# hellobertrand/zxc

Measured on NVIDIA H100. Metric: decompress GB/s (uncompressed), higher is better.
Workload: dtype u8

## Files before the change

include/zxc_b200.h:

```cpp
#ifndef ZXC_B200_H
#define ZXC_B200_H

#include <stddef.h>
#include <stdint.h>

#include "zxc_export.h"
#include "zxc_opts.h"

#ifdef __cplusplus
extern "C" {
#endif

typedef struct {
    uint64_t src_off;
    uint64_t dst_off;
    uint32_t src_len;
    uint32_t dst_cap;
} zxc_b200_job_t;

typedef struct {
    uint64_t decoded_size;
    uint32_t block_size;
    uint32_t n_blocks;
    uint32_t dict_id;
// ... 12 lines not shown
ZXC_EXPORT int zxc_b200_decode_blocks(const void* d_src, void* d_dst, const zxc_b200_job_t* d_jobs,
                                      uint32_t n_jobs, int32_t* d_status, const void* d_dict,
                                      uint32_t dict_size, const void* d_dict_huf, void* d_scratch,
                                      size_t scratch_size, uint32_t block_size,
                                      int verify_checksums, void* stream);

ZXC_EXPORT int64_t zxc_b200_reduce_status(const int32_t* d_status, const zxc_b200_job_t* d_jobs,
                                          uint32_t n_jobs, void* stream);

ZXC_EXPORT size_t zxc_b200_encode_scratch_size(uint64_t src_size, const zxc_compress_opts_t* opts);

ZXC_EXPORT int zxc_b200_compress_device(const void* d_src, uint64_t src_size, void* d_dst, uint64_t dst_capacity,
                                        const zxc_compress_opts_t* opts, void* d_scratch, size_t scratch_size,
                                        int64_t* d_result, zxc_b200_job_t* d_jobs, void* stream);

ZXC_EXPORT size_t zxc_b200_decompress_device_scratch_size(uint64_t dst_capacity, uint32_t block_size);

ZXC_EXPORT int zxc_b200_decompress_device(const void* d_src, uint64_t src_size, void* d_dst, uint64_t dst_capacity,
                                          const zxc_decompress_opts_t* opts, void* d_scratch, size_t scratch_size,
                                          int64_t* d_result, void* stream);

ZXC_EXPORT uint64_t zxc_b200_launch_count(void);

ZXC_EXPORT int zxc_b200_train_phase_times(double* ms, int n);

#ifdef __cplusplus
}
#endif
#endif
```

profiles/occupancy_probe.py:

```python
import argparse
import ctypes as C
import os
import re
import shutil
import subprocess
import sys
import tempfile
import time

ROOT = os.path.dirname(os.path.dirname(os.path.abspath(__file__)))
sys.path.insert(0, os.path.join(ROOT, "tests"))
sys.path.insert(0, ROOT)

VARIANTS = [
    ("parent", "parent", "", {}, "baseline: lean at 7 CTAs, 72 registers"),
    ("pad7", "pad7", "-DLEAN_SMEM_PAD=2048u", {}, "7 CTAs, 164 KB carve-out: the L1 shrink alone"),
    ("reg64_7", "reg64_7", "-DLEAN_CTAS_PER_SM=8u -DLEAN_CARVEOUT=57", {},
     "64-register build, 132 KB carve-out hint, so 7 CTAs if the driver follows the hint: the spills alone"),
    ("cta8", "cta8", "-DLEAN_CTAS_PER_SM=8u", {}, "8 CTAs, 64 registers, 164 KB carve-out: both"),
    ("cta8_grid7", "cta8", "-DLEAN_CTAS_PER_SM=8u", {"ZXC_B200_DECODE_CTAS": "7"},
     "the 8-CTA build with a 7-CTA grid: spills and the L1 shrink, without the eighth CTA"),
    ("parent_grid6", "parent", "", {"ZXC_B200_DECODE_CTAS": "6"}, "the lean instance's own 6 -> 7 CTA step"),
    ("ring2k_7", "ring2k_7", "-DRING_BYTES=2048u", {}, "7 CTAs, 2 KiB rings"),
    ("ring2k_8", "ring2k_8", "-DRING_BYTES=2048u -DLEAN_CTAS_PER_SM=8u", {},
     "8 CTAs, 2 KiB rings: more warps at a 100 KB carve-out"),
]
LEAN = "_Z17zxc_decode_kernelILb0ELb0ELb0ELb1EEv12DecodeParams"


def build(out_dir, nvextra):
    lib = os.path.join(out_dir, "libzxc.so.4")
    if not os.path.exists(lib):
        subprocess.run(["make", "-j", str(os.cpu_count() or 4), f"NVEXTRA={nvextra}", f"OUT={out_dir}"],
                       cwd=os.path.join(ROOT, "zxc_b200", "csrc"), check=True, stdout=subprocess.DEVNULL)
    return lib


def lean_resources(out_dir):
    log = open(os.path.join(out_dir, "obj", "ptxas.log")).read()
    blk = log.split(f"Compiling entry function '{LEAN}'")[1].split("Compiling entry function")[0]
    sp = re.search(r"(\d+) bytes spill stores, (\d+) bytes spill loads", blk)
    return int(re.search(r"Used (\d+) registers", blk).group(1)), int(sp.group(1)), int(sp.group(2))


def card():
    q = "name,power.limit,clocks.max.sm,clocks.sm"
    r = subprocess.run(["nvidia-smi", f"--query-gpu={q}", "--format=csv,noheader"], stdout=subprocess.PIPE, text=True)
    return r.stdout.strip().splitlines()[0] if r.returncode == 0 and r.stdout.strip() else "nvidia-smi unavailable"


class Runner:
    def __init__(self, path, dev, d_src, d_dst, d_jobs, d_status, nb):
        import bench
        import torch

        lib = C.CDLL(path)
        lib.zxc_b200_decode_scratch_size.restype = C.c_size_t
        lib.zxc_b200_decode_scratch_size.argtypes = [C.c_uint32]
        lib.zxc_b200_decode_blocks.restype = C.c_int
        lib.zxc_b200_decode_blocks.argtypes = [C.c_void_p, C.c_void_p, C.c_void_p, C.c_uint32, C.c_void_p,
                                               C.c_void_p, C.c_uint32, C.c_void_p, C.c_void_p, C.c_size_t,
                                               C.c_uint32, C.c_int, C.c_void_p]
        self.lib, self.nb, self.block = lib, nb, bench.BLOCK
        self.bufs = (d_src, d_dst, d_jobs, d_status)
        self.scratch_size = lib.zxc_b200_decode_scratch_size(bench.BLOCK)
        self.d_scratch = torch.empty(self.scratch_size, dtype=torch.uint8, device=dev)
        self.stream = torch.cuda.current_stream(dev)

    def step(self):
        d_src, d_dst, d_jobs, d_status = self.bufs
        rc = self.lib.zxc_b200_decode_blocks(d_src.data_ptr(), d_dst.data_ptr(), d_jobs.data_ptr(), self.nb,
                                             d_status.data_ptr(), None, 0, None, self.d_scratch.data_ptr(),
                                             self.scratch_size, self.block, 0, self.stream.cuda_stream)
        assert rc == 0, rc

    def time(self, steps):
        import torch

        e0, e1 = torch.cuda.Event(enable_timing=True), torch.cuda.Event(enable_timing=True)
        e0.record(self.stream)
        for _ in range(steps):
            self.step()
        e1.record(self.stream)
        e1.synchronize()
        return e0.elapsed_time(e1) / steps


def main():
    ap = argparse.ArgumentParser()
    ap.add_argument("--out", help="build directory (default: a temporary one)")
# ... 34 lines not shown
    prod.zxc_b200_plan_frame.restype = C.c_int64
    prod.zxc_b200_plan_frame.argtypes = [C.c_void_p, C.c_size_t, C.c_void_p, C.c_size_t, C.c_void_p]
    nb = prod.zxc_b200_plan_frame(frame.ctypes.data, frame.size, None, 0, None)
    jobs = np.zeros(nb * C.sizeof(bench.Job), dtype=np.uint8)
    assert prod.zxc_b200_plan_frame(frame.ctypes.data, frame.size, jobs.ctypes.data, nb, None) == nb
    dev = torch.device("cuda", 0)
    d_src = torch.from_numpy(frame).to(dev)
    d_dst = torch.empty(data.size, dtype=torch.uint8, device=dev)
    d_jobs = torch.from_numpy(jobs).to(dev)
    d_status = torch.empty(nb, dtype=torch.int32, device=dev)
    want = torch.from_numpy(data).to(dev)
    runners = {}
    for name, _, _, env, _ in variants:
        r = Runner(libs[name], dev, d_src, d_dst, d_jobs, d_status, nb)
        d_dst.zero_()
        os.environ.update(env)
        for _ in range(3):
            r.step()
        torch.cuda.synchronize(dev)
        for k in env:
            del os.environ[k]
        assert torch.equal(d_dst, want), f"{name}: decoded bytes differ"
        runners[name] = r
    del want
    rates = {v[0]: [] for v in variants}
    for k in range(args.rounds):
        for name in rates:
            runners[name].time(2)
            ms = runners[name].time(args.steps)
            rates[name].append(data.size / ms / 1e6)
        print(f"round {k + 1}: " + ", ".join(f"{n} {rates[n][-1]:.1f}" for n in rates), flush=True)
        time.sleep(0.5)
    print(f"\ncard after the runs: {card()}")
    base = np.median(rates[variants[0][0]])
    print(f"\n| variant | GB/s decoded, per round | median | spread | against {variants[0][0]} |")
    print("|---|---|---|---|---|")
    for name in rates:
        v = rates[name]
        med = float(np.median(v))
        print(f"| {name} | {' / '.join(f'{x:.1f}' for x in v)} | {med:.1f} | {100 * (max(v) - min(v)) / med:.2f} % | "
              f"{100 * (med / base - 1):+.1f} % |")


if __name__ == "__main__":
    main()
```

zxc_b200/csrc/zxc_decode.cuh:

```cuda
#pragma once
#include <cuda_runtime.h>
#include <stdint.h>

#include "zxc_b200.h"
#include "zxc_error.h"

typedef uint8_t u8;
typedef uint32_t u32;
typedef uint64_t u64;
typedef int32_t i32;

#define FULL 0xFFFFFFFFu
#ifndef ZXC_FASTMOD
#define ZXC_FASTMOD 1
#endif
#ifndef ZXC_TAIL_SMEM
#define ZXC_TAIL_SMEM 1
#endif
#ifndef ZXC_ALIGNED_LD
#define ZXC_ALIGNED_LD 1
#endif
#ifndef ZXC_HINTS
#define ZXC_HINTS 0
#endif
#if ZXC_HINTS
#define ZXC_RARE(x) __builtin_expect(!!(x), 0)
#else
#define ZXC_RARE(x) (x)
#endif
#ifndef ZXC_STAT
#define ZXC_STAT(i, v)
#endif
#ifndef WARPS_PER_CTA
#define WARPS_PER_CTA 4
#endif
#define CTA_THREADS (WARPS_PER_CTA * 32)
#ifndef RING_BYTES
#define RING_BYTES 4096u
#endif
#define RING_LIMIT (RING_BYTES - 576u)
#ifndef CTAS_PER_SM
#define CTAS_PER_SM 7u
#endif
#ifndef LEAN_CTAS_PER_SM
#define LEAN_CTAS_PER_SM CTAS_PER_SM
#endif
#ifndef LEAN_SMEM_PAD
#define LEAN_SMEM_PAD 0u
#endif

#define BT_RAW 0
#define BT_GLO 1
#define BT_GHI 2
#define BT_EOF 255

#define FLAG_VERIFY 1u
#define FLAG_UNITS_ON 4u
#define FLAG_UNITS_OFF 8u
#define FLAG_DEFERRED 2u
#define D2_DEFER_STATUS ((i32)0x80000000)

struct DecodeParams {
    const u8* src;
    u8* dst;
    const zxc_b200_job_t* jobs;
    i32* status;
    const u8* dict;
    const u8* dict_huf;
    u8* scratch;
    unsigned long long* counter;
    u32 n_jobs;
    u32 dict_size;
    u32 scratch_stride;
    u32 flags;
    u32 block_cap;
    u32* defer_list;
    u32* defer_count;
    u32 defer_cap;
};

__device__ __forceinline__ u32 ld16(const u8* p) { return (u32)p[0] | ((u32)p[1] << 8); }
__device__ __forceinline__ u32 ld32(const u8* p) {
    return (u32)p[0] | ((u32)p[1] << 8) | ((u32)p[2] << 16) | ((u32)p[3] << 24);
}
__device__ __forceinline__ u64 ld64(const u8* p) { return (u64)ld32(p) | ((u64)ld32(p + 4) << 32); }

__device__ __forceinline__ u32 warp_incl_scan(u32 v, u32 lane) {
#pragma unroll
    for (int d = 1; d < 32; d <<= 1) {
        const u32 t = __shfl_up_sync(FULL, v, d);
        if (lane >= (u32)d) v += t;
    }
    return v;
}

#ifdef __CUDACC__
__device__ __forceinline__ u32 smem_addr(const void* p) {
    u32 a = (u32)__cvta_generic_to_shared(p);
    asm volatile("" : "+r"(a));
    return a;
}
template <int OFF> __device__ __forceinline__ void sts32(u32 a, u32 v) {
    asm volatile("st.shared.u32 [%0+%2], %1;" ::"r"(a), "r"(v), "n"(OFF) : "memory");
}
template <int OFF> __device__ __forceinline__ void sts16(u32 a, u32 v) {
    asm volatile("st.shared.u16 [%0+%2], %1;" ::"r"(a), "h"((unsigned short)v), "n"(OFF) : "memory");
}
template <int OFF> __device__ __forceinline__ void sts8(u32 a, u32 v) {
    asm volatile("st.shared.u8 [%0+%2], %1;" ::"r"(a), "r"(v), "n"(OFF) : "memory");
}
#else
extern u8 smem[];
static inline u32 smem_addr(const void* p) { return (u32)(reinterpret_cast<const u8*>(p) - smem); }
template <int OFF> static inline void sts32(u32 a, u32 v) { memcpy(smem + a + OFF, &v, 4); }
template <int OFF> static inline void sts16(u32 a, u32 v) { const unsigned short h = (unsigned short)v; memcpy(smem + a + OFF, &h, 2); }
template <int OFF> static inline void sts8(u32 a, u32 v) { smem[a + OFF] = (u8)v; }
#endif

#ifdef __CUDACC__
__device__ __forceinline__ void prefetch_l1(const void* p) { asm volatile("prefetch.global.L1 [%0];" ::"l"(p)); }
#else
static inline void prefetch_l1(const void*) {}
#endif

#if ZXC_TRACE
#define TRACE_SLOTS 16
#define TRACE_ROWS 8192
enum {
    TR_UNPACK, TR_SCAN, TR_LIT, TR_MATCH, TR_TAIL, TR_FLUSH, TR_START, TR_END, TR_GIANT, TR_CLAIM,
    TR_BATCHES, TR_BLOCKS, TR_M_RING, TR_M_GLOBAL, TR_M_DICT, TR_M_SEQ
};
__device__ unsigned long long zxc_trace_acc[TRACE_ROWS * TRACE_SLOTS];
__device__ __forceinline__ void trace_add(u32 slot, unsigned long long v, u32 lane) {
    const u32 row = blockIdx.x * WARPS_PER_CTA + (threadIdx.x >> 5);
    if (lane == 0 && row < TRACE_ROWS) atomicAdd(&zxc_trace_acc[row * TRACE_SLOTS + slot], v);
}
// ... 215 lines not shown
                if (lit_comp > avail) return ZXC_ERROR_CORRUPT_DATA;
                const int rc = rle_expand(p_data, lit_comp, scratch, n_lit, lane);
                if (rc != ZXC_OK) return rc;
                __syncwarp();
                S.lit = scratch;
                S.n_lit_avail = n_lit;
            } else {
                S.lit = p_data;
                S.n_lit_avail = 0;
            }
        } else if (enc_lit == 0) {
            S.lit = p_data;
            S.n_lit_avail = lit_comp;
        } else {
            return ZXC_ERROR_CORRUPT_DATA;
        }
        const u64 sz_off = enc_off ? (u64)n_seq : (u64)n_seq * 2;
        const u64 consumed = (u64)lit_comp + tok_comp + sz_off;
        if (consumed > avail) return ZXC_ERROR_CORRUPT_DATA;
        if (avail - lit_comp < 32) return ZXC_ERROR_CORRUPT_DATA;
        if (enc_tok != 0 && enc_tok != 2) return ZXC_ERROR_CORRUPT_DATA;
        S.tok = p_data + lit_comp;
        S.offs = S.tok + tok_comp;
        if (!LEAN && enc_tok == 2) {
            if (n_seq == 0 || n_seq > block_cap / 5u + 16u || tok_comp < 128) return ZXC_ERROR_CORRUPT_DATA;
            const int rc = pivco_decode(S.tok, S.tok + 128, tok_comp - 128, tok_buf, n_seq, hw, cum, cum_words, lane);
            if (rc != ZXC_OK) return rc;
            __syncwarp();
            S.tok = tok_buf;
        }
        S.ext = S.offs + (u32)sz_off;
        S.ext_end = avail - (u32)consumed;
    } else {
        if (enc_lit != 0 || enc_tok != 0) return ZXC_ERROR_CORRUPT_DATA;
        const u32 avail = comp - 12;
        const u64 consumed = (u64)n_lit + (u64)n_seq * 4;
        if (consumed > avail) return ZXC_ERROR_CORRUPT_DATA;
        if (avail - n_lit < 32) return ZXC_ERROR_CORRUPT_DATA;
        S.lit = pay + 12;
        S.n_lit_avail = n_lit;
        S.tok = S.lit + n_lit;
        S.ext = S.tok + (size_t)n_seq * 4;
        S.ext_end = avail - (u32)consumed;
    }
    return ZXC_OK;
}
// ... 209 lines not shown
            const u32 m = (u32)(reinterpret_cast<uintptr_t>(bp)) & 3u;
            const u32* wp = reinterpret_cast<const u32*>(bp - m) + w0;
            const u32 dw = ring_s + (pj & 0xFFFFu) - da + 4u * w0;
            const u32 sh = m * 8u;
            const u32 left = lfe - w0;
            const u32 nsrc = left + (m ? 1u : 0u);
            u32 W[5];
#pragma unroll
            for (int i = 0; i < 5; i++) W[i] = (u32)i < nsrc ? wp[i] : 0u;
            sts32<0>(dw, __funnelshift_r(W[0], W[1], sh));
            if (1 < left) sts32<4>(dw, __funnelshift_r(W[1], W[2], sh));
            if (2 < left) sts32<8>(dw, __funnelshift_r(W[2], W[3], sh));
            if (3 < left) sts32<12>(dw, __funnelshift_r(W[3], W[4], sh));
        }
    }
}

#ifndef ZXC_NW
#define ZXC_NW 8
#endif
#define LIT_SHORT (4u * ZXC_NW - 4u)
#define MATCH_SHORT (4u * ZXC_NW - 4u)

template <bool UNITS, bool GHI, bool HAS_DICT, bool LEAN>
__device__ int decode_lz_block(const u8* pay, u32 comp, u8* out, u32 cap, const u8* dict_in,
                               u32 dict_size_in, const u8* dict_huf, u8* scratch, u32 scratch_cap, u8* ring,
                               u32 lane, u32 P_flags) {
    constexpr bool ghi = GHI;
    const u8* dict = HAS_DICT ? dict_in : (const u8*)0;
    const u32 dict_size = HAS_DICT ? dict_size_in : 0u;
    ZXC_TRACE_DECL;
    ZXC_TRACE_ADD(TR_BLOCKS, 1, lane);
    Sections S;
    const int prc = parse_sections<LEAN>(pay, comp, ghi, cap, dict_huf, scratch, scratch_cap, lane, S);
    if (prc != ZXC_OK) return prc;
    const u8* lit = S.lit;
    const u8* tok = S.tok;
    const u8* offs = S.offs;
    const u8* ext = S.ext;
    const u32 ext_end = S.ext_end, n_lit_avail = S.n_lit_avail, n_seq = S.n_seq, enc_off = S.enc_off;

    (void)P_flags;
    if (UNITS && cap <= 65536u) {
        u8* tok_buf = scratch + scr_lit_cap(scratch_cap);
        u8* hw_area = tok_buf + scr_tok_cap(scratch_cap);
        const bool scratch_busy = (lit == scratch) || (tok == tok_buf);
        u8* tab = scratch_busy ? hw_area : scratch;
        const u32 tab_bytes = scratch_busy ? (u32)HUF_WORK_BYTES + scr_cum_cap(scratch_cap)
                                           : scr_stride(scratch_cap) - 256u;
        const int r = decode_lz_units(lit, n_lit_avail, tok, offs, ext, ext_end, n_seq, enc_off, ghi, out, cap, dict,
                                      dict_size, tab, tab_bytes, lane);
        if (r != UW_NOT_TAKEN) return r;
    }

    const u32 mask = RING_BYTES - 1;
    const u32 esc = ghi ? 255u : 15u;
    const u32 lt_mask = (1u << lane) - 1u;
    const bool al16 = (reinterpret_cast<uintptr_t>(out) & 15u) == 0;
    Window w;
    w.ring = ring;
    w.out = out;
    w.dict = dict;
    w.dict_size = dict_size;
    w.near_lo = 0;
    const u32 ring_s = smem_addr(ring);
    (void)ring_s;
    u32 O = 0, L = 0, F = 0, epos = 0, ring_lo = 0;

    u32* vals = reinterpret_cast<u32*>(scratch + scr_lit_cap(scratch_cap) + scr_tok_cap(scratch_cap) + (u32)HUF_WORK_BYTES);
    if constexpr (LEAN) {
        if (4ull * ext_end > scr_cum_cap(scratch_cap)) return D2_DEFER_STATUS;
    }
    const bool use_vals = LEAN || (ext_end != 0u && 4ull * ext_end <= scr_cum_cap(scratch_cap));
    u32 n_val = 0, ord_base = 0;
    if (use_vals && (!LEAN || ext_end != 0u)) {
        const u32 seg = max(4u, (ext_end + 31u) / 32u);
        const u32 nseg = (ext_end + seg - 1u) / seg;
        const u32 lo = lane * seg, hi = min(ext_end, lo + seg);
        u64 inc = lane < nseg ? z2_seg_map(ext, lo, hi, ext_end) : Z2_MAP_ID;
#pragma unroll
        for (int dd = 1; dd < 32; dd <<= 1) {
            const u64 o = __shfl_up_sync(FULL, inc, dd);
            if (lane >= (u32)dd) inc = z2_map_compose(o, inc);
        }
        u64 excl = __shfl_up_sync(FULL, inc, 1);
        if (lane == 0) excl = Z2_MAP_ID;
        n_val = z2_map_cnt(__shfl_sync(FULL, inc, 31), 0);
        if (lane < nseg) {
            const u32 ent = z2_map_exit(excl, 0);
            if (ent != 3u) z2_seg_values(ext, lo, hi, ext_end, ent, z2_map_cnt(excl, 0), vals);
        }
        __syncwarp();
// ... 45 lines not shown
                    b = enc_off ? (u32)offs[i] : ld16(offs + 2 * (size_t)i);
                } else if (enc_off) {
                    b = lds8(st_o.ring_s + ((ox0 + i) & (ST_RING - 1u)));
                } else {
                    const u32 x = ox0 + 2u * i;
                    b = (ox0 & 1u) ? (lds8(st_o.ring_s + (x & (ST_RING - 1u))) |
                                      (lds8(st_o.ring_s + ((x + 1u) & (ST_RING - 1u))) << 8))
                                   : lds16(st_o.ring_s + (x & (ST_RING - 1u)));
                }
            } else if (t_st) {
                const u32 x = tx0 + 4u * i;
                if (tx0 & 3u) {
                    a = lds8(st_t.ring_s + (x & (ST_RING - 1u))) | (lds8(st_t.ring_s + ((x + 1u) & (ST_RING - 1u))) << 8) |
                        (lds8(st_t.ring_s + ((x + 2u) & (ST_RING - 1u))) << 16) |
                        (lds8(st_t.ring_s + ((x + 3u) & (ST_RING - 1u))) << 24);
                } else {
                    a = lds32(st_t.ring_s + (x & (ST_RING - 1u)));
                }
            } else {
                a = ld32(tok + 4 * (size_t)i);
            }
#else
            if (!ghi) {
                a = tok[i];
#if ZXC_ALIGNED_LD
                if (LEAN) {
                    const u32 oi = n_seq + (enc_off ? i : 2u * i);
                    if (enc_off) b = (u32)tok[oi];
                    else if ((reinterpret_cast<uintptr_t>(tok) + n_seq) & 1u) b = ld16(tok + oi);
                    else b = (u32)*reinterpret_cast<const unsigned short*>(tok + oi);
                } else if (enc_off) b = (u32)offs[i];
                else if (reinterpret_cast<uintptr_t>(offs) & 1u) b = ld16(offs + 2 * (size_t)i);
                else b = (u32)reinterpret_cast<const unsigned short*>(offs)[i];
#else
                b = enc_off ? (u32)offs[i] : ld16(offs + 2 * (size_t)i);
#endif
            } else {
#if ZXC_ALIGNED_LD
                a = (reinterpret_cast<uintptr_t>(tok) & 3u) ? ld32(tok + 4 * (size_t)i) : reinterpret_cast<const u32*>(tok)[i];
#else
                a = ld32(tok + 4 * (size_t)i);
#endif
            }
#endif
            if (!ghi) {
                ll = a >> 4;
                ml = a & 15;
                off = b + 1;
            } else {
                ll = a >> 24;
                ml = (a >> 16) & 0xFF;
                off = (a & 0xFFFF) + 1;
            }
        }
        const bool e_ll = valid && ll == esc, e_ml = valid && ml == esc;
        const u32 m_ll = __ballot_sync(FULL, e_ll), m_ml = __ballot_sync(FULL, e_ml);
        ZXC_TRACE_MARK(TR_UNPACK, lane);
        u32 k_esc = 0, epos_end = epos;
        if ((m_ll | m_ml) && use_vals) {
            u32 k = ord_base + __popc(m_ll & lt_mask) + __popc(m_ml & lt_mask);
            if (e_ll) {
                ll += k < n_val ? vals[k] : 0u;
                k++;
            }
            if (e_ml) ml += k < n_val ? vals[k] : 0u;
        } else if (ZXC_RARE((m_ll | m_ml) != 0)) {
            const u32 ord_ll = __popc(m_ll & lt_mask) + __popc(m_ml & lt_mask);
            k_esc = __popc(m_ll) + __popc(m_ml);
            u32 my_pos = ext_end;
            for (u32 s = 0; s < k_esc; s++) {
                if (s == ord_ll) my_pos = epos_end;
                epos_end = varint_advance(ext, epos_end, ext_end);
            }
            if (e_ll) ll += read_varint(ext, my_pos, ext_end);
            if (e_ml) ml += read_varint(ext, my_pos, ext_end);
        }
        if (valid) ml += 5;
        const u32 tot = ll + ml;
        const u32 s_ll = warp_incl_scan(ll, lane);
        const u32 s_tot = warp_incl_scan(tot, lane);

        const u32 nvalid = min(32u, n_seq - base);
        const u32 m = __popc(__ballot_sync(FULL, valid && s_tot <= RING_LIMIT));
        const u32 lit_start = L + s_ll - ll;
        const u32 out_start = O + s_tot - tot;
        const u32 mdst = out_start + ll;

        if (ZXC_RARE(m == 0)) {
            const u32 g_ll = __shfl_sync(FULL, ll, 0), g_ml = __shfl_sync(FULL, ml, 0),
                      g_off = __shfl_sync(FULL, off, 0);
            ZXC_STAT(9, 1);
            if (L + g_ll > n_lit_avail || (u64)O + g_ll + g_ml > cap) {
                ST_CLOSE();
                return ZXC_ERROR_OVERFLOW;
            }
            if (O + g_ll + dict_size < g_off) {
                ST_CLOSE();
                return ZXC_ERROR_BAD_OFFSET;
            }
            __syncwarp();
            ring_flush(w, F, O, lane, al16);
            __syncwarp();
            flush_wait(lane);
            warp_copy(out + O, lit + L, g_ll, lane);
            __syncwarp();
            warp_match_global(w, O + g_ll, g_off, g_ml, lane);
            __syncwarp();
            O += g_ll + g_ml;
            L += g_ll;
            F = O;
            ring_lo = O >= 64 ? O - 64 : 0;
            for (u32 p = ring_lo + lane; p < O; p += 32) ring[p & mask] = out[p];
            __syncwarp();
            const u32 q = ((m_ll & 1u) ? 1u : 0u) + ((m_ml & 1u) ? 1u : 0u);
            ord_base += q;
            if (!use_vals)
                for (u32 s = 0; s < q; s++) epos = varint_advance(ext, epos, ext_end);
            base += 1;
            ZXC_TRACE_MARK(TR_GIANT, lane);
            continue;
        }

        ZXC_STAT(10, m < nvalid);
        ZXC_STAT(11, m < nvalid && !use_vals);
        const bool act = lane < m;
        const bool ovf = act && (lit_start + ll > n_lit_avail || out_start + tot > cap);
        const bool bad = act && (mdst + dict_size < off);
        const u32 m_err = __ballot_sync(FULL, ovf || bad);
        if (ZXC_RARE(m_err != 0)) {
            ZXC_STAT(19, 1);
            const int code = ovf ? ZXC_ERROR_OVERFLOW : ZXC_ERROR_BAD_OFFSET;
            ST_CLOSE();
            return __shfl_sync(FULL, code, __ffs(m_err) - 1);
        }
        const u32 T = __shfl_sync(FULL, s_tot, m - 1), TL = __shfl_sync(FULL, s_ll, m - 1);
#if ZXC_STAGE && ZXC_STAGE_LIT
        const u32 lx0 = (u32)(reinterpret_cast<uintptr_t>(lit) & 15u);
        const StWindow lw = LitStream::need(stage_s, lit, lx0 + L, lx0 + L + TL, 8u, lane);
#endif
        {
            const i32 a = (i32)(O + T) - (i32)RING_BYTES + 32;
            w.near_lo = a > (i32)ring_lo ? a : (i32)ring_lo;
        }

        flush_wait(lane);
        const i32 src_lo = (i32)mdst - (i32)off;
        const i32 src_end = min((i32)mdst, src_lo + (i32)ml);
        const bool near = src_lo >= w.near_lo;
        const u32 si = (u32)src_lo & mask;
        const bool in_dict = src_lo + (i32)ml + 8 <= 0 && (i32)dict_size + src_lo >= 8;
        const bool m_word_ok = ((mdst & mask) + ml + 4 <= RING_BYTES) &&
                               (near ? (si >= 8 && si + ml + 8 <= RING_BYTES)
                                     : (in_dict || (src_lo >= 8 && src_lo + (i32)ml + 4 <= w.near_lo)));
        const bool m_lane_ok = m_word_ok && ml <= MATCH_SHORT && off >= ml;
        const bool m_grp_ok = m_word_ok && !m_lane_ok && off >= ml;
        const u8* m_sp = near ? ring + si : (src_lo < 0 ? dict + ((i32)dict_size + src_lo) : out + src_lo);
        const bool l_word_ok = (out_start & mask) + ll + 4 <= RING_BYTES;

        const bool m_free = src_end <= (i32)O;
        if (LEAN && !HAS_DICT && act && m_free && !near && src_lo >= 0) {
            const u8* ps = out + src_lo;
            const u8* pe = ps + ml - 1u;
            prefetch_l1(ps);
            if ((reinterpret_cast<uintptr_t>(ps) ^ reinterpret_cast<uintptr_t>(pe)) >> 7) prefetch_l1(pe);
        }
        ZXC_TRACE_ADD(TR_M_RING, __popc(__ballot_sync(FULL, act && near)), lane);
        ZXC_TRACE_ADD(TR_M_GLOBAL, __popc(__ballot_sync(FULL, act && !near && src_lo >= 0)), lane);
        ZXC_TRACE_ADD(TR_M_DICT, __popc(__ballot_sync(FULL, act && !near && src_lo < 0)), lane);
        ZXC_TRACE_ADD(TR_M_SEQ, __popc(__ballot_sync(FULL, act && !m_free)), lane);
        ZXC_TRACE_ADD(TR_BATCHES, 1, lane);
        ZXC_TRACE_MARK(TR_SCAN, lane);
        ZXC_STAT(0, 1);
        ZXC_STAT(1, m);
        bool lit_pass = true;
#pragma unroll 1
        for (;;) {
            bool ready, lok, gok;
            u32 it_d, it_n;
            const u8* it_sp;
            if (lit_pass) {
                ready = act && ll > 0;
                it_d = out_start;
                it_n = ll;
                it_sp = lit + lit_start;
#if ZXC_STAGE && ZXC_STAGE_LIT
                {
                    const u8* sp_s = lit_ptr(lw, lx0 + lit_start, ll);
                    if (sp_s) it_sp = sp_s;
                    ZXC_STAT(13, __popc(__ballot_sync(FULL, ready && sp_s != 0)));
                    ZXC_STAT(14, __popc(__ballot_sync(FULL, ready)));
                }
#endif
                lok = l_word_ok && ll <= LIT_SHORT;
                gok = l_word_ok && ll > LIT_SHORT;
            } else {
                ready = act && m_free;
                it_d = mdst;
                it_n = ml;
                it_sp = m_sp;
                lok = m_lane_ok;
                gok = m_grp_ok;
            }
            lane_copy_words2<ZXC_NW>(ring_s, it_d, it_sp, it_n, ready && lok);
            const u32 m_grp = __ballot_sync(FULL, ready && gok);
            ZXC_STAT(2, 1);
            ZXC_STAT(3, __popc(__ballot_sync(FULL, ready && lok)));
            ZXC_STAT(4, __popc(m_grp));
            ZXC_STAT(5, m_grp != 0);
            ZXC_STAT(6, __popc(__ballot_sync(FULL, ready && !lok && !gok)));
            ZXC_STAT(7, __ballot_sync(FULL, ready && lok) != 0);
            ZXC_STAT(17, __popc(__ballot_sync(FULL, !lit_pass && ready && (lok || gok) && src_lo < 0)));
            ZXC_STAT(18, __popc(__ballot_sync(FULL, !lit_pass && ready && !lok && !gok)));
            ZXC_STAT(20, __popc(__ballot_sync(FULL, !lit_pass && ready && (lok || gok) && near)));
            ZXC_STAT(21, __popc(__ballot_sync(FULL, !lit_pass && ready && (lok || gok) && !near && src_lo >= 0)));
            if (m_grp) balanced_copy_words(ring_s, m_grp, it_d, it_sp, it_n, lane);
            u32 m_slow = __ballot_sync(FULL, ready && !lok && !gok);
            while (ZXC_RARE(m_slow != 0)) {
                const int j = __ffs(m_slow) - 1;
                m_slow &= m_slow - 1;
                const u32 d = __shfl_sync(FULL, it_d, j), n = __shfl_sync(FULL, it_n, j);
                const u32 aux = __shfl_sync(FULL, lit_pass ? lit_start : off, j);
                if (lit_pass) {
                    for (u32 k = lane; k < n; k += 32) ring[(d + k) & mask] = lit[aux + k];
                } else {
                    warp_match_to_ring(w, d, aux, n, lane);
                }
            }
            __syncwarp();
            ZXC_TRACE_MARK(lit_pass ? TR_LIT : TR_MATCH, lane);
            if (!lit_pass) break;
            lit_pass = false;
        }
        {
            u32 rest = __ballot_sync(FULL, act && !m_free);
            const u32 my_pk = ml | ((near && off >= ml) ? 0x80000000u : 0u);
            ZXC_STAT(12, __popc(rest));
            while (rest) {
                const int j = __ffs(rest) - 1;
                rest &= rest - 1;
                const u32 d = __shfl_sync(FULL, mdst, j), pk = __shfl_sync(FULL, my_pk, j);
                const u32 n = pk & 0x7FFFFFFFu;
                if (pk >> 31) {
                    const u32 sl = __shfl_sync(FULL, (u32)src_lo, j);
#if ZXC_TAIL_SMEM
                    for (u32 k = lane; k < n; k += 32) sts8<0>(ring_s + ((d + k) & mask), lds8(ring_s + ((sl + k) & mask)));
#else
                    for (u32 k = lane; k < n; k += 32) ring[(d + k) & mask] = ring[(sl + k) & mask];
#endif
                } else {
                    warp_match_to_ring(w, d, __shfl_sync(FULL, off, j), n, lane);
                }
                __syncwarp();
            }
        }
        ZXC_TRACE_MARK(TR_TAIL, lane);

        O += T;
        L += TL;
        ring_flush(w, F, O & ~511u, lane, al16);
        __syncwarp();
        ZXC_TRACE_MARK(TR_FLUSH, lane);

        if (m < nvalid) {
            const u32 below = (1u << m) - 1u;
            const u32 q = __popc(m_ll & below) + __popc(m_ml & below);
            ord_base += q;
            if (!use_vals)
                for (u32 s = 0; s < q; s++) epos = varint_advance(ext, epos, ext_end);
            base += m;
        } else {
            ord_base += __popc(m_ll) + __popc(m_ml);
            epos = epos_end;
            base += 32;
        }
    }

    ST_LIT_CLOSE();
    const u32 rem = n_lit_avail - L;
    if (rem > cap - O) return ZXC_ERROR_OVERFLOW;
    ring_flush(w, F, O, lane, al16);
    __syncwarp();
    flush_wait(lane);
    warp_copy(out + O, lit + L, rem, lane);
    ZXC_TRACE_MARK(TR_END, lane);
    return (int)(O + rem);
}

template <bool UNITS, bool HAS_DICT, bool LEAN = false>
__device__ int decode_job(const DecodeParams& P, const zxc_b200_job_t& job, u8* scratch, u8* ring, u32 lane) {
    const u8* blk = P.src + job.src_off;
    u8* out = P.dst + job.dst_off;
    if (job.src_len < 8) return LEAN ? D2_DEFER_STATUS : ZXC_ERROR_SRC_TOO_SMALL;
    const u32 type = blk[0];
    const u32 comp = ld32(blk + 3);
    const bool verify = (P.flags & FLAG_VERIFY) != 0;
    if (LEAN) {
        const bool whole = !verify && (u64)job.src_len >= 8ull + comp;
        const bool take = whole && (type == BT_RAW || (type == BT_GLO && comp >= 12u && blk[8 + 9] == 0 && blk[8 + 8] <= 1));
        if (!take) return D2_DEFER_STATUS;
    }
    if ((u64)job.src_len < 8ull + comp + (verify ? 4u : 0u)) return ZXC_ERROR_SRC_TOO_SMALL;
    const u8* data = blk + 8;
    if constexpr (!LEAN) {
        if (verify && ld32(data + comp) != warp_checksum(data, comp, lane)) return ZXC_ERROR_BAD_CHECKSUM;
    }
    switch (type) {
        case BT_GLO:
            return decode_lz_block<UNITS, false, HAS_DICT, LEAN>(data, comp, out, job.dst_cap, P.dict, P.dict_size,
                                                                 P.dict_huf, scratch, P.block_cap, ring, lane, P.flags);
        case BT_GHI:
            if constexpr (LEAN) return D2_DEFER_STATUS;
            else return decode_lz_block<UNITS, true, HAS_DICT, false>(data, comp, out, job.dst_cap, P.dict, P.dict_size,
                                                                      P.dict_huf, scratch, P.block_cap, ring, lane, P.flags);
        case BT_RAW:
            if (comp > job.dst_cap) return ZXC_ERROR_DST_TOO_SMALL;
            warp_copy(out, data, comp, lane);
            return (int)comp;
        case BT_EOF:
            return ZXC_ERROR_CORRUPT_DATA;
        default:
            return ZXC_ERROR_BAD_BLOCK_TYPE;
    }
}

template <bool UNITS, bool DEFERRED, bool HAS_DICT, bool LEAN>
__global__ void __launch_bounds__(CTA_THREADS, LEAN ? LEAN_CTAS_PER_SM : CTAS_PER_SM) zxc_decode_kernel(const DecodeParams P) {
    extern __shared__ __align__(16) u8 smem[];
    const u32 lane = threadIdx.x & 31;
    const u32 wic = threadIdx.x >> 5;
    const u32 gwarp = blockIdx.x * WARPS_PER_CTA + wic;
    u8* scratch = P.scratch + (size_t)gwarp * P.scratch_stride + 256;
    u8* ring = smem + (size_t)wic * WARP_SMEM_BYTES;
#if ZXC_STAGE
    st_init(smem_addr(ring) + RING_BYTES, lane);
#endif
    if (DEFERRED) {
        const u32 n_def = *P.defer_count;
        if (n_def == 0) return;
        if (n_def <= P.defer_cap) {
            for (;;) {
                unsigned long long k = 0;
                if (lane == 0) k = atomicAdd(P.counter, 1ull);
                k = __shfl_sync(FULL, k, 0);
                if (k >= n_def) break;
                const u32 j = P.defer_list[k];
                const zxc_b200_job_t job = P.jobs[j];
                const int r = decode_job<UNITS, HAS_DICT, false>(P, job, scratch, ring, lane);
                flush_wait(lane);
                __syncwarp();
                if (lane == 0) P.status[j] = r;
            }
            return;
        }
        for (;;) {
            unsigned long long b = 0;
            if (lane == 0) b = atomicAdd(P.counter, 32ull);
            b = __shfl_sync(FULL, b, 0);
            if (b >= P.n_jobs) break;
            const unsigned long long jj = b + lane;
            u32 m = __ballot_sync(FULL, jj < P.n_jobs && P.status[jj] == D2_DEFER_STATUS);
            while (m) {
                const unsigned long long j = b + (u32)(__ffs(m) - 1);
                m &= m - 1;
                const zxc_b200_job_t job = P.jobs[j];
                const int r = decode_job<UNITS, HAS_DICT, false>(P, job, scratch, ring, lane);
                flush_wait(lane);
                __syncwarp();
                if (lane == 0) P.status[j] = r;
            }
        }
        return;
    }
    for (;;) {
        ZXC_TRACE_DECL;
        unsigned long long j = 0;
        if (lane == 0) j = atomicAdd(P.counter, 1ull);
        j = __shfl_sync(FULL, j, 0);
        ZXC_TRACE_MARK(TR_CLAIM, lane);
        if (j >= P.n_jobs) break;
        const zxc_b200_job_t job = P.jobs[j];
        const int r = decode_job<UNITS, HAS_DICT, LEAN>(P, job, scratch, ring, lane);
        flush_wait(lane);
        __syncwarp();
        if (lane == 0) {
            P.status[j] = r;
            if (LEAN && r == D2_DEFER_STATUS) {
                const u32 slot = atomicAdd(P.defer_count, 1u);
                if (slot < P.defer_cap) P.defer_list[slot] = (u32)j;
            }
        }
    }
}

__global__ void zxc_reduce_kernel(const i32* status, const zxc_b200_job_t* jobs, u32 n,
                                  unsigned long long* out ) {
    const u32 i = blockIdx.x * blockDim.x + threadIdx.x;
    unsigned long long bad = ~0ull, sum = 0;
    if (i < n) {
        const i32 s = status[i];
        if (s < 0 || (u32)s != jobs[i].dst_cap) bad = i;
        else sum = (u32)s;
    }
    for (int d = 16; d >= 1; d >>= 1) {
        const unsigned long long ob = __shfl_xor_sync(FULL, bad, d);
// ... 9 lines not shown
```

zxc_b200/csrc/zxc_gpu.cu:

```cuda
#include <cuda_runtime.h>
#include <stdint.h>
#include <stdio.h>
#include <stdlib.h>
#include <string.h>
#include <pthread.h>

#include "zxc_error.h"
#include "zxc_gpu.h"

#include "zxc_decode.cuh"
#include "zxc_decode2.cuh"
#include "zxc_encode.cuh"
#include "zxc_assemble.cuh"
#include "zxc_dplan.cuh"
#include "zxc_train.cuh"

static pthread_once_t g_once = PTHREAD_ONCE_INIT;
static int g_init_rc = ZXC_B200_ERROR_NO_DEVICE;
static int g_sm_count = 0;
static unsigned long long g_launches = 0;
static pthread_mutex_t g_pool_mu = PTHREAD_MUTEX_INITIALIZER;

#define PIN_CHUNK ((size_t)32 << 20)

// ... 256 lines not shown
    int dev = 0;
    cudaGetDevice(&dev);
    cudaDeviceProp prop;
    if (cudaGetDeviceProperties(&prop, dev) != cudaSuccess) {
        g_init_rc = ZXC_B200_ERROR_CUDA;
        return;
    }
    g_sm_count = prop.multiProcessorCount;
    g_init_rc = ZXC_OK;
}

extern "C" int zxg_init(void) {
    pthread_once(&g_once, init_once);
    return g_init_rc;
}

extern "C" int zxc_b200_device_count(void) {
    int n = 0;
    if (cudaGetDeviceCount(&n) != cudaSuccess) return 0;
    return n;
}

extern "C" uint64_t zxc_b200_launch_count(void) { return g_launches; }

#if ZXC_TRACE
extern "C" ZXC_EXPORT int zxc_b200_trace_read(unsigned long long* host) {
    const size_t bytes = sizeof(unsigned long long) * TRACE_ROWS * TRACE_SLOTS;
    if (cudaDeviceSynchronize() != cudaSuccess) return -1;
    if (cudaMemcpyFromSymbol(host, zxc_trace_acc, bytes) != cudaSuccess) return -1;
    void* d = 0;
    if (cudaGetSymbolAddress(&d, zxc_trace_acc) != cudaSuccess || cudaMemset(d, 0, bytes) != cudaSuccess) return -1;
    if (cudaDeviceSynchronize() != cudaSuccess) return -1;
    return TRACE_ROWS * TRACE_SLOTS;
}
#endif

extern "C" int zxg_current_device(void) {
    int dev = 0;
    if (cudaGetDevice(&dev) != cudaSuccess) {
        cudaGetLastError();
        return 0;
    }
    return dev;
}
extern "C" int zxg_device_count(void) { return zxc_b200_device_count(); }
extern "C" int zxg_set_device(int dev) {
// ... 279 lines not shown
    P.src = (const u8*)d_src;
    P.dst = (u8*)d_dst;
    P.jobs = d_jobs;
    P.status = d_status;
    P.dict = (const u8*)d_dict;
    P.dict_huf = (const u8*)d_dict_huf;
    P.scratch = (u8*)d_scratch;
    P.counter = d_counter;
    P.n_jobs = n_jobs;
    P.dict_size = d_dict ? dict_size : 0;
    P.scratch_stride = scratch_stride_for(block_size);
    P.flags = verify ? FLAG_VERIFY : 0;
    {
        static int units_mode = -2;
        if (units_mode == -2) {
            const char* e = getenv("ZXC_B200_UNITS");
            units_mode = e ? (e[0] == '1' ? 1 : 0) : -1;
        }
        if (units_mode == 1) P.flags |= FLAG_UNITS_ON;
        if (units_mode == 0) P.flags |= FLAG_UNITS_OFF;
    }
    const bool units = (P.flags & FLAG_UNITS_ON) != 0;
    P.block_cap = block_size;
    const int grid = grid_for(n_jobs);
    const size_t warp_scratch = (size_t)grid * WARPS_PER_CTA * P.scratch_stride;
    if (warp_scratch > scratch_size) return ZXC_ERROR_MEMORY;
    if (!preset && cudaMemsetAsync(d_counter, 0, 3 * sizeof(unsigned long long), st) != cudaSuccess)
        return ZXC_B200_ERROR_CUDA;
    size_t off = (warp_scratch + 255) & ~(size_t)255;
    P.defer_count = (u32*)(d_counter + 2);
    P.defer_cap = off + (size_t)DEFER_CAP * 4 <= scratch_size ? DEFER_CAP : 0u;
    P.defer_list = (u32*)((u8*)d_scratch + off);
    D2Config c;
    if (!verify && d2_config(block_size, &c)) {
        static int attr_done_smem = 0;
        if (attr_done_smem < (int)c.smem) {
            if (cudaFuncSetAttribute(zxc_decode2_kernel, cudaFuncAttributeMaxDynamicSharedMemorySize, 233472 - 1024) !=
                cudaSuccess)
                return ZXC_B200_ERROR_CUDA;
            attr_done_smem = 233472;
        }
        Decode2Params Q;
        Q.src = P.src;
        Q.dst = P.dst;
        Q.jobs = d_jobs;
        Q.status = d_status;
        Q.dict = P.dict;
// ... 55 lines not shown
        }
        P.flags |= FLAG_DEFERRED;
        P.counter = d_counter + 1;
    }
    const bool has_dict = P.dict != NULL && P.dict_size != 0;
    if (!verify && !units && !(P.flags & FLAG_DEFERRED)) {
#ifdef LEAN_CARVEOUT
        static int carveout_done = 0;
        if (!carveout_done) {
            cudaFuncSetAttribute(zxc_decode_kernel<false, false, true, true>,
                                 cudaFuncAttributePreferredSharedMemoryCarveout, LEAN_CARVEOUT);
            cudaFuncSetAttribute(zxc_decode_kernel<false, false, false, true>,
                                 cudaFuncAttributePreferredSharedMemoryCarveout, LEAN_CARVEOUT);
            carveout_done = 1;
        }
#endif
        const u32 lean_smem = DECODE_SMEM_BYTES + LEAN_SMEM_PAD;
        if (has_dict) zxc_decode_kernel<false, false, true, true><<<grid, CTA_THREADS, lean_smem, st>>>(P);
        else zxc_decode_kernel<false, false, false, true><<<grid, CTA_THREADS, lean_smem, st>>>(P);
        __atomic_add_fetch(&g_launches, 1, __ATOMIC_RELAXED);
        if (cudaGetLastError() != cudaSuccess) return ZXC_B200_ERROR_CUDA;
        P.flags |= FLAG_DEFERRED;
        P.counter = d_counter + 1;
    }
    if (P.flags & FLAG_DEFERRED) {
        if (has_dict) zxc_decode_kernel<false, true, true, false><<<grid, CTA_THREADS, DECODE_SMEM_BYTES, st>>>(P);
        else zxc_decode_kernel<false, true, false, false><<<grid, CTA_THREADS, DECODE_SMEM_BYTES, st>>>(P);
    } else if (units) {
        if (has_dict) zxc_decode_kernel<true, false, true, false><<<grid, CTA_THREADS, DECODE_SMEM_BYTES, st>>>(P);
        else zxc_decode_kernel<true, false, false, false><<<grid, CTA_THREADS, DECODE_SMEM_BYTES, st>>>(P);
    } else {
        if (has_dict) zxc_decode_kernel<false, false, true, false><<<grid, CTA_THREADS, DECODE_SMEM_BYTES, st>>>(P);
        else zxc_decode_kernel<false, false, false, false><<<grid, CTA_THREADS, DECODE_SMEM_BYTES, st>>>(P);
    }
    __atomic_add_fetch(&g_launches, 1, __ATOMIC_RELAXED);
    return cudaGetLastError() == cudaSuccess ? ZXC_OK : ZXC_B200_ERROR_CUDA;
}

static int launch_decode(const void* d_src, void* d_dst, const zxc_b200_job_t* d_jobs, u32 n_jobs,
                         i32* d_status, const void* d_dict, u32 dict_size, const void* d_dict_huf,
                         void* d_scratch, size_t scratch_size, u32 block_size, int verify,
                         unsigned long long* d_counter, cudaStream_t st) {
    return launch_decode_ex(d_src, d_dst, d_jobs, n_jobs, d_status, d_dict, dict_size, d_dict_huf, d_scratch,
                            scratch_size, block_size, verify, d_counter, st, 0);
}

// ... 1046 lines not shown
```

Baseline: 395.0.

## Run lean decode kernel at 8 CTAs per SM by trimming live registers

Raises the lean decode kernel's launch bound from 7 to 8 CTAs per SM. To fit the tighter register budget without spills, it recomputes the scratch pointer, ring pointer and escape table from tid/ctaid at their point of use instead of keeping them live, hiding them behind opaque asm. It also copies tokens next to the literals in scratch so one base pointer addresses both, narrows the job index to 32 bits, and caps the general kernel's grid at its resident CTA count. This adds recomputation and an extra token copy per block, and risks spills or a shrunken L1 in exchange for more resident warps.

```diff
diff --git a/include/zxc_b200.h b/include/zxc_b200.h
--- a/include/zxc_b200.h
+++ b/include/zxc_b200.h
@@ -58,6 +58,8 @@
 
 ZXC_EXPORT uint64_t zxc_b200_launch_count(void);
 
+ZXC_EXPORT int zxc_b200_decode_occupancy(int* lean, int* general);
+
 ZXC_EXPORT int zxc_b200_train_phase_times(double* ms, int n);
 
 #ifdef __cplusplus
diff --git a/profiles/occupancy_probe.py b/profiles/occupancy_probe.py
--- a/profiles/occupancy_probe.py
+++ b/profiles/occupancy_probe.py
@@ -13,17 +13,14 @@
 sys.path.insert(0, ROOT)
 
 VARIANTS = [
-    ("parent", "parent", "", {}, "baseline: lean at 7 CTAs, 72 registers"),
-    ("pad7", "pad7", "-DLEAN_SMEM_PAD=2048u", {}, "7 CTAs, 164 KB carve-out: the L1 shrink alone"),
-    ("reg64_7", "reg64_7", "-DLEAN_CTAS_PER_SM=8u -DLEAN_CARVEOUT=57", {},
-     "64-register build, 132 KB carve-out hint, so 7 CTAs if the driver follows the hint: the spills alone"),
-    ("cta8", "cta8", "-DLEAN_CTAS_PER_SM=8u", {}, "8 CTAs, 64 registers, 164 KB carve-out: both"),
-    ("cta8_grid7", "cta8", "-DLEAN_CTAS_PER_SM=8u", {"ZXC_B200_DECODE_CTAS": "7"},
-     "the 8-CTA build with a 7-CTA grid: spills and the L1 shrink, without the eighth CTA"),
-    ("parent_grid6", "parent", "", {"ZXC_B200_DECODE_CTAS": "6"}, "the lean instance's own 6 -> 7 CTA step"),
-    ("ring2k_7", "ring2k_7", "-DRING_BYTES=2048u", {}, "7 CTAs, 2 KiB rings"),
-    ("ring2k_8", "ring2k_8", "-DRING_BYTES=2048u -DLEAN_CTAS_PER_SM=8u", {},
-     "8 CTAs, 2 KiB rings: more warps at a 100 KB carve-out"),
+    ("parent", "parent", "", {}, "shipped: lean at 8 CTAs, 64 registers without spills"),
+    ("cta7", "cta7", "-DLEAN_CTAS_PER_SM=7u", {}, "the same source built for 7 CTAs (72 registers)"),
+    ("grid7", "parent", "", {"ZXC_B200_DECODE_CTAS": "7"},
+     "the shipped build with a 7-CTA grid: the eighth CTA alone, at the 164 KB carve-out"),
+    ("pad7", "pad7", "-DLEAN_CTAS_PER_SM=7u -DLEAN_SMEM_PAD=2048u", {},
+     "7 CTAs, 164 KB carve-out: the L1 shrink alone"),
+    ("ring2k_7", "ring2k_7", "-DRING_BYTES=2048u -DLEAN_CTAS_PER_SM=7u", {}, "7 CTAs, 2 KiB rings"),
+    ("ring2k_8", "ring2k_8", "-DRING_BYTES=2048u", {}, "8 CTAs, 2 KiB rings: more warps at a 100 KB carve-out"),
 ]
 LEAN = "_Z17zxc_decode_kernelILb0ELb0ELb0ELb1EEv12DecodeParams"
 
@@ -66,6 +63,9 @@
         self.scratch_size = lib.zxc_b200_decode_scratch_size(bench.BLOCK)
         self.d_scratch = torch.empty(self.scratch_size, dtype=torch.uint8, device=dev)
         self.stream = torch.cuda.current_stream(dev)
+        lean, general = C.c_int(0), C.c_int(0)
+        assert lib.zxc_b200_decode_occupancy(C.byref(lean), C.byref(general)) == 0
+        self.occupancy = (lean.value, general.value)
 
     def step(self):
         d_src, d_dst, d_jobs, d_status = self.bufs
@@ -146,6 +146,7 @@
             del os.environ[k]
         assert torch.equal(d_dst, want), f"{name}: decoded bytes differ"
         runners[name] = r
+        print(f"{name}: resident CTAs per SM, lean / general instance: {r.occupancy[0]} / {r.occupancy[1]}", flush=True)
     del want
     rates = {v[0]: [] for v in variants}
     for k in range(args.rounds):
diff --git a/zxc_b200/csrc/zxc_decode.cuh b/zxc_b200/csrc/zxc_decode.cuh
--- a/zxc_b200/csrc/zxc_decode.cuh
+++ b/zxc_b200/csrc/zxc_decode.cuh
@@ -1,6 +1,8 @@
 #pragma once
 #include <cuda_runtime.h>
 #include <stdint.h>
+
+#include <type_traits>
 
 #include "zxc_b200.h"
 #include "zxc_error.h"
@@ -43,7 +45,7 @@
 #define CTAS_PER_SM 7u
 #endif
 #ifndef LEAN_CTAS_PER_SM
-#define LEAN_CTAS_PER_SM CTAS_PER_SM
+#define LEAN_CTAS_PER_SM 8u
 #endif
 #ifndef LEAN_SMEM_PAD
 #define LEAN_SMEM_PAD 0u
@@ -79,6 +81,10 @@
     u32 defer_cap;
 };
 
+__host__ __device__ __forceinline__ u8* warp_scratch(const DecodeParams& P, u32 gwarp) {
+    return P.scratch + (size_t)gwarp * P.scratch_stride + 256;
+}
+
 __device__ __forceinline__ u32 ld16(const u8* p) { return (u32)p[0] | ((u32)p[1] << 8); }
 __device__ __forceinline__ u32 ld32(const u8* p) {
     return (u32)p[0] | ((u32)p[1] << 8) | ((u32)p[2] << 16) | ((u32)p[3] << 24);
@@ -109,9 +115,23 @@
 template <int OFF> __device__ __forceinline__ void sts8(u32 a, u32 v) {
     asm volatile("st.shared.u8 [%0+%2], %1;" ::"r"(a), "r"(v), "n"(OFF) : "memory");
 }
+__device__ __forceinline__ u32 opaque(u32 v) {
+    asm volatile("" : "+r"(v));
+    return v;
+}
+__device__ __forceinline__ u8* ring_at(u32 a) { return reinterpret_cast<u8*>(__cvta_shared_to_generic((size_t)opaque(a))); }
+__device__ __forceinline__ u32 grid_warp_now() {
+    u32 t, c;
+    asm volatile("mov.u32 %0, %%tid.x;" : "=r"(t));
+    asm volatile("mov.u32 %0, %%ctaid.x;" : "=r"(c));
+    return c * WARPS_PER_CTA + (t >> 5);
+}
 #else
 extern u8 smem[];
 static inline u32 smem_addr(const void* p) { return (u32)(reinterpret_cast<const u8*>(p) - smem); }
+static inline u32 opaque(u32 v) { return v; }
+static inline u8* ring_at(u32 a) { return smem + a; }
+static inline u32 grid_warp_now() { return blockIdx.x * WARPS_PER_CTA + (threadIdx.x >> 5); }
 template <int OFF> static inline void sts32(u32 a, u32 v) { memcpy(smem + a + OFF, &v, 4); }
 template <int OFF> static inline void sts16(u32 a, u32 v) { const unsigned short h = (unsigned short)v; memcpy(smem + a + OFF, &h, 2); }
 template <int OFF> static inline void sts8(u32 a, u32 v) { smem[a + OFF] = (u8)v; }
@@ -373,6 +393,15 @@
         if (enc_tok != 0 && enc_tok != 2) return ZXC_ERROR_CORRUPT_DATA;
         S.tok = p_data + lit_comp;
         S.offs = S.tok + tok_comp;
+        if (LEAN && S.lit == scratch) {
+            const u32 ts = tok_comp + (u32)sz_off;
+            if ((u64)n_lit + ts > scratch_cap + scr_tok_cap(block_cap) + (u32)HUF_WORK_BYTES) return D2_DEFER_STATUS;
+            warp_copy(scratch + n_lit, S.tok, ts, lane);
+            __syncwarp();
+            S.tok = scratch + n_lit;
+        } else if (LEAN && S.n_lit_avail == 0) {
+            S.lit = S.tok;
+        }
         if (!LEAN && enc_tok == 2) {
             if (n_seq == 0 || n_seq > block_cap / 5u + 16u || tok_comp < 128) return ZXC_ERROR_CORRUPT_DATA;
             const int rc = pivco_decode(S.tok, S.tok + 128, tok_comp - 128, tok_buf, n_seq, hw, cum, cum_words, lane);
@@ -628,10 +657,14 @@
 #define LIT_SHORT (4u * ZXC_NW - 4u)
 #define MATCH_SHORT (4u * ZXC_NW - 4u)
 
+__device__ __forceinline__ u32* esc_table(u8* scratch, u32 block_cap) {
+    return reinterpret_cast<u32*>(scratch + scr_lit_cap(block_cap) + scr_tok_cap(block_cap) + (u32)HUF_WORK_BYTES);
+}
+
 template <bool UNITS, bool GHI, bool HAS_DICT, bool LEAN>
 __device__ int decode_lz_block(const u8* pay, u32 comp, u8* out, u32 cap, const u8* dict_in,
                                u32 dict_size_in, const u8* dict_huf, u8* scratch, u32 scratch_cap, u8* ring,
-                               u32 lane, u32 P_flags) {
+                               u32 lane, const DecodeParams& P) {
     constexpr bool ghi = GHI;
     const u8* dict = HAS_DICT ? dict_in : (const u8*)0;
     const u32 dict_size = HAS_DICT ? dict_size_in : 0u;
@@ -646,7 +679,6 @@
     const u8* ext = S.ext;
     const u32 ext_end = S.ext_end, n_lit_avail = S.n_lit_avail, n_seq = S.n_seq, enc_off = S.enc_off;
 
-    (void)P_flags;
     if (UNITS && cap <= 65536u) {
         u8* tok_buf = scratch + scr_lit_cap(scratch_cap);
         u8* hw_area = tok_buf + scr_tok_cap(scratch_cap);
@@ -671,9 +703,13 @@
     w.near_lo = 0;
     const u32 ring_s = smem_addr(ring);
     (void)ring_s;
+#define W_RING()                                     \
+    do {                                             \
+        if constexpr (LEAN) w.ring = ring_at(ring_s); \
+    } while (0)
     u32 O = 0, L = 0, F = 0, epos = 0, ring_lo = 0;
 
-    u32* vals = reinterpret_cast<u32*>(scratch + scr_lit_cap(scratch_cap) + scr_tok_cap(scratch_cap) + (u32)HUF_WORK_BYTES);
+    u32* vals = esc_table(scratch, scratch_cap);
     if constexpr (LEAN) {
         if (4ull * ext_end > scr_cum_cap(scratch_cap)) return D2_DEFER_STATUS;
     }
@@ -765,13 +801,15 @@
             }
 #else
             if (!ghi) {
-                a = tok[i];
+                const u8* tk = tok;
+                if constexpr (LEAN) tk = lit + opaque(n_lit_avail);
+                a = tk[i];
 #if ZXC_ALIGNED_LD
                 if (LEAN) {
                     const u32 oi = n_seq + (enc_off ? i : 2u * i);
-                    if (enc_off) b = (u32)tok[oi];
-                    else if ((reinterpret_cast<uintptr_t>(tok) + n_seq) & 1u) b = ld16(tok + oi);
-                    else b = (u32)*reinterpret_cast<const unsigned short*>(tok + oi);
+                    if (enc_off) b = (u32)tk[oi];
+                    else if ((reinterpret_cast<uintptr_t>(tk) + n_seq) & 1u) b = ld16(tk + oi);
+                    else b = (u32)*reinterpret_cast<const unsigned short*>(tk + oi);
                 } else if (enc_off) b = (u32)offs[i];
                 else if (reinterpret_cast<uintptr_t>(offs) & 1u) b = ld16(offs + 2 * (size_t)i);
                 else b = (u32)reinterpret_cast<const unsigned short*>(offs)[i];
@@ -801,12 +839,14 @@
         ZXC_TRACE_MARK(TR_UNPACK, lane);
         u32 k_esc = 0, epos_end = epos;
         if ((m_ll | m_ml) && use_vals) {
+            const u32* vt = vals;
+            if constexpr (LEAN) vt = esc_table(warp_scratch(P, grid_warp_now()), P.block_cap);
             u32 k = ord_base + __popc(m_ll & lt_mask) + __popc(m_ml & lt_mask);
             if (e_ll) {
-                ll += k < n_val ? vals[k] : 0u;
+                ll += k < n_val ? vt[k] : 0u;
                 k++;
             }
-            if (e_ml) ml += k < n_val ? vals[k] : 0u;
+            if (e_ml) ml += k < n_val ? vt[k] : 0u;
         } else if (ZXC_RARE((m_ll | m_ml) != 0)) {
             const u32 ord_ll = __popc(m_ll & lt_mask) + __popc(m_ml & lt_mask);
             k_esc = __popc(m_ll) + __popc(m_ml);
@@ -842,6 +882,7 @@
                 return ZXC_ERROR_BAD_OFFSET;
             }
             __syncwarp();
+            W_RING();
             ring_flush(w, F, O, lane, al16);
             __syncwarp();
             flush_wait(lane);
@@ -853,7 +894,7 @@
             L += g_ll;
             F = O;
             ring_lo = O >= 64 ? O - 64 : 0;
-            for (u32 p = ring_lo + lane; p < O; p += 32) ring[p & mask] = out[p];
+            for (u32 p = ring_lo + lane; p < O; p += 32) w.ring[p & mask] = out[p];
             __syncwarp();
             const u32 q = ((m_ll & 1u) ? 1u : 0u) + ((m_ml & 1u) ? 1u : 0u);
             ord_base += q;
@@ -897,7 +938,11 @@
                                      : (in_dict || (src_lo >= 8 && src_lo + (i32)ml + 4 <= w.near_lo)));
         const bool m_lane_ok = m_word_ok && ml <= MATCH_SHORT && off >= ml;
         const bool m_grp_ok = m_word_ok && !m_lane_ok && off >= ml;
-        const u8* m_sp = near ? ring + si : (src_lo < 0 ? dict + ((i32)dict_size + src_lo) : out + src_lo);
+        auto match_src = [&]() -> const u8* {
+            return near ? (LEAN ? ring_at(ring_s + si) : ring + si)
+                        : (src_lo < 0 ? dict + ((i32)dict_size + src_lo) : out + src_lo);
+        };
+        const u8* m_sp = LEAN ? nullptr : match_src();
         const bool l_word_ok = (out_start & mask) + ll + 4 <= RING_BYTES;
 
         const bool m_free = src_end <= (i32)O;
@@ -940,7 +985,7 @@
                 ready = act && m_free;
                 it_d = mdst;
                 it_n = ml;
-                it_sp = m_sp;
+                it_sp = LEAN ? match_src() : m_sp;
                 lok = m_lane_ok;
                 gok = m_grp_ok;
             }
@@ -963,8 +1008,9 @@
                 m_slow &= m_slow - 1;
                 const u32 d = __shfl_sync(FULL, it_d, j), n = __shfl_sync(FULL, it_n, j);
                 const u32 aux = __shfl_sync(FULL, lit_pass ? lit_start : off, j);
+                W_RING();
                 if (lit_pass) {
-                    for (u32 k = lane; k < n; k += 32) ring[(d + k) & mask] = lit[aux + k];
+                    for (u32 k = lane; k < n; k += 32) w.ring[(d + k) & mask] = lit[aux + k];
                 } else {
                     warp_match_to_ring(w, d, aux, n, lane);
                 }
@@ -991,6 +1037,7 @@
                     for (u32 k = lane; k < n; k += 32) ring[(d + k) & mask] = ring[(sl + k) & mask];
 #endif
                 } else {
+                    W_RING();
                     warp_match_to_ring(w, d, __shfl_sync(FULL, off, j), n, lane);
                 }
                 __syncwarp();
@@ -1000,6 +1047,7 @@
 
         O += T;
         L += TL;
+        W_RING();
         ring_flush(w, F, O & ~511u, lane, al16);
         __syncwarp();
         ZXC_TRACE_MARK(TR_FLUSH, lane);
@@ -1021,6 +1069,8 @@
     ST_LIT_CLOSE();
     const u32 rem = n_lit_avail - L;
     if (rem > cap - O) return ZXC_ERROR_OVERFLOW;
+    W_RING();
+#undef W_RING
     ring_flush(w, F, O, lane, al16);
     __syncwarp();
     flush_wait(lane);
@@ -1050,11 +1100,11 @@
     switch (type) {
         case BT_GLO:
             return decode_lz_block<UNITS, false, HAS_DICT, LEAN>(data, comp, out, job.dst_cap, P.dict, P.dict_size,
-                                                                 P.dict_huf, scratch, P.block_cap, ring, lane, P.flags);
+                                                                 P.dict_huf, scratch, P.block_cap, ring, lane, P);
         case BT_GHI:
             if constexpr (LEAN) return D2_DEFER_STATUS;
             else return decode_lz_block<UNITS, true, HAS_DICT, false>(data, comp, out, job.dst_cap, P.dict, P.dict_size,
-                                                                      P.dict_huf, scratch, P.block_cap, ring, lane, P.flags);
+                                                                      P.dict_huf, scratch, P.block_cap, ring, lane, P);
         case BT_RAW:
             if (comp > job.dst_cap) return ZXC_ERROR_DST_TOO_SMALL;
             warp_copy(out, data, comp, lane);
@@ -1072,7 +1122,7 @@
     const u32 lane = threadIdx.x & 31;
     const u32 wic = threadIdx.x >> 5;
     const u32 gwarp = blockIdx.x * WARPS_PER_CTA + wic;
-    u8* scratch = P.scratch + (size_t)gwarp * P.scratch_stride + 256;
+    u8* scratch = warp_scratch(P, gwarp);
     u8* ring = smem + (size_t)wic * WARP_SMEM_BYTES;
 #if ZXC_STAGE
     st_init(smem_addr(ring) + RING_BYTES, lane);
@@ -1114,15 +1164,19 @@
         }
         return;
     }
+    using JobIx = typename std::conditional<LEAN, u32, unsigned long long>::type;
+    u32 ring_s = 0;
+    if constexpr (LEAN) ring_s = smem_addr(ring);
     for (;;) {
         ZXC_TRACE_DECL;
-        unsigned long long j = 0;
-        if (lane == 0) j = atomicAdd(P.counter, 1ull);
-        j = __shfl_sync(FULL, j, 0);
+        unsigned long long c = 0;
+        if (lane == 0) c = atomicAdd(P.counter, 1ull);
+        const JobIx j = __shfl_sync(FULL, (JobIx)c, 0);
         ZXC_TRACE_MARK(TR_CLAIM, lane);
         if (j >= P.n_jobs) break;
         const zxc_b200_job_t job = P.jobs[j];
-        const int r = decode_job<UNITS, HAS_DICT, LEAN>(P, job, scratch, ring, lane);
+        const int r = LEAN ? decode_job<UNITS, HAS_DICT, LEAN>(P, job, warp_scratch(P, grid_warp_now()), ring_at(ring_s), lane)
+                           : decode_job<UNITS, HAS_DICT, LEAN>(P, job, scratch, ring, lane);
         flush_wait(lane);
         __syncwarp();
         if (lane == 0) {
diff --git a/zxc_b200/csrc/zxc_gpu.cu b/zxc_b200/csrc/zxc_gpu.cu
--- a/zxc_b200/csrc/zxc_gpu.cu
+++ b/zxc_b200/csrc/zxc_gpu.cu
@@ -302,6 +302,16 @@
 }
 
 extern "C" uint64_t zxc_b200_launch_count(void) { return g_launches; }
+
+extern "C" int zxc_b200_decode_occupancy(int* lean, int* general) {
+    if (zxg_init() != ZXC_OK) return ZXC_B200_ERROR_CUDA;
+    if (cudaOccupancyMaxActiveBlocksPerMultiprocessor(lean, zxc_decode_kernel<false, false, false, true>, CTA_THREADS,
+                                                      DECODE_SMEM_BYTES + LEAN_SMEM_PAD) != cudaSuccess ||
+        cudaOccupancyMaxActiveBlocksPerMultiprocessor(general, zxc_decode_kernel<false, true, false, false>, CTA_THREADS,
+                                                      DECODE_SMEM_BYTES) != cudaSuccess)
+        return ZXC_B200_ERROR_CUDA;
+    return ZXC_OK;
+}
 
 #if ZXC_TRACE
 extern "C" ZXC_EXPORT int zxc_b200_trace_read(unsigned long long* host) {
@@ -627,7 +637,7 @@
     }
     const bool units = (P.flags & FLAG_UNITS_ON) != 0;
     P.block_cap = block_size;
-    const int grid = grid_for(n_jobs);
+    int grid = grid_for(n_jobs);
     const size_t warp_scratch = (size_t)grid * WARPS_PER_CTA * P.scratch_stride;
     if (warp_scratch > scratch_size) return ZXC_ERROR_MEMORY;
     if (!preset && cudaMemsetAsync(d_counter, 0, 3 * sizeof(unsigned long long), st) != cudaSuccess)
@@ -729,6 +739,10 @@
         if (cudaGetLastError() != cudaSuccess) return ZXC_B200_ERROR_CUDA;
         P.flags |= FLAG_DEFERRED;
         P.counter = d_counter + 1;
+    }
+    {
+        const int resident = (g_sm_count > 0 ? g_sm_count : 132) * (int)CTAS_PER_SM;
+        if (grid > resident) grid = resident;
     }
     if (P.flags & FLAG_DEFERRED) {
         if (has_dict) zxc_decode_kernel<false, true, true, false><<<grid, CTA_THREADS, DECODE_SMEM_BYTES, st>>>(P);
```

Result: faster. 429.9, median of 6 (+8.8%).
